# JingyunLiang/HCFlow

Measured on AMD Instinct MI355X. Metric: HR images/sec (inverse sample) DIV2K x4 160px LR, higher is better.
Workload: dtype f32 via f16x3 split (hi/lo f16 products, f32 accumulate); 1 GPU; SR_DF2K_4X inverse sampling (netG reverse=True), batch 16/GPU, LR 160x160 -> HR 640x640, tau=0.8, eps on device, output all-gather over RCCL for N>1; global_batch=16, lr_size=160, parallelism=dp1, streams_per_gpu=2

## Files before the change

### hcflow_amd/_lib.py

```python
from __future__ import annotations

import ctypes as C
import os
from typing import List, Optional, Sequence, Tuple

import torch

_HERE = os.path.dirname(os.path.abspath(__file__))
LIB_PATH = os.environ.get("HCFLOW_LIB", os.path.join(_HERE, "libhcflow_hip.so"))

HCF_OK = 0
ERR_NAMES = {-1: "HCF_ERR_ARG", -2: "HCF_ERR_HIP", -3: "HCF_ERR_STATE", -4: "HCF_ERR_KEY",
             -5: "HCF_ERR_SHAPE", -6: "HCF_ERR_UNSUPPORTED", -7: "HCF_ERR_NOMEM"}
FLAG_NO_CLAMP = 1
FLAG_NO_RANGE_CHECK = 2
FLAG_KEEP_COND = 4
FLAG_REUSE_COND = 8
DATA_LAUNCH_BATCH = 64

SYMBOLS = [
    "hcf_create", "hcf_destroy", "hcf_last_error", "hcf_param_count", "hcf_param_info",
    "hcf_set_param", "hcf_finalize", "hcf_inverse", "hcf_inverse_ex", "hcf_check_range", "hcf_check_range_samples", "hcf_aux_stream", "hcf_forward_sr", "hcf_forward_rescale",
    "hcf_encode_sr",
    "hcf_workspace_bytes", "hcf_weight_bytes", "hcf_profile_convs", "hcf_conv_time_ms",
# ... 5 lines not shown
    "hcf_train_forward_sr", "hcf_train_backward", "hcf_train_backward_phase", "hcf_bind_param_device", "hcf_refresh_from_device",
    "hcf_train_inverse", "hcf_train_backward_inverse", "hcf_metric_psnr_ssim", "hcf_metric_imresize_down",
    "hcf_train_select_tape", "hcf_train_forward_rescale", "hcf_train_backward_rescale",
    "hcf_debug_range_probe", "hcf_debug_range_probe_read", "hcf_debug_conv_plan",
    "hcf_aux_conv2d_workspace", "hcf_aux_conv2d", "hcf_aux_conv2d_backward", "hcf_adam_step",
    "hcf_lpips_workspace", "hcf_lpips_alex", "hcf_lpips_backward_workspace", "hcf_lpips_alex_backward",
    "hcf_aux_bn_act_workspace", "hcf_aux_bn_act", "hcf_aux_bn_act_backward",
    "hcf_op_step_forward_backward", "hcf_op_step_inverse_backward", "hcf_op_prior_backward", "hcf_op_quant_logp_backward",
    "hcf_op_output_grad_backward", "hcf_op_conv_epilogue_backward", "hcf_op_lu_chain",
    "hcf_train_backward_inverse_ex", "hcf_train_backward_counts", "hcf_op_prior_sample_backward",
    "hcf_aux_input_norm", "hcf_aux_input_norm_backward", "hcf_aux_maxpool2", "hcf_aux_maxpool2_act_backward",
    "hcf_aux_act_backward", "hcf_aux_feature_loss_workspace", "hcf_aux_feature_loss",
    "hcf_train_backward_ex", "hcf_train_backward_rescale_ex", "hcf_train_encode_sr", "hcf_train_backward_encode",
    "hcf_op_quant_logp_backward_lr", "hcf_op_prior_encode_logp_backward", "hcf_op_input_grad",
    "hcf_data_prepare_batch", "hcf_data_prepare_paired",
    "hcf_op_fcn12", "hcf_op_conv2d_step_inverse",
]


class HcfError(RuntimeError):
    pass


class hcf_config(C.Structure):
    _fields_ = [
        ("kind", C.c_int32), ("scale", C.c_int32), ("in_nc", C.c_int32), ("quant", C.c_float),
        ("L", C.c_int32), ("K", C.c_int32 * 4), ("after", C.c_int32 * 4), ("squeeze", C.c_int32),
        ("perm", C.c_int32), ("coupling", C.c_int32), ("nn_module", C.c_int32), ("hidden", C.c_int32),
        ("c_perm", C.c_int32), ("c_coupling", C.c_int32), ("c_nn_module", C.c_int32), ("c_hidden", C.c_int32),
        ("rrdb_nb", C.c_int32 * 2), ("rrdb_nf", C.c_int32), ("rrdb_gc", C.c_int32),
        ("lu_decomposed", C.c_int32),
# ... 90 lines not shown
    lib.hcf_refresh_from_device.argtypes = [vp, vp]
    lib.hcf_train_forward_sr.argtypes = [vp, fp, fp, fp, fp, fp, fp, i32, i32, i32, vp]
    lib.hcf_train_backward.argtypes = [vp, f32, fp, i64, vp]
    lib.hcf_train_backward_phase.argtypes = [vp, i32, f32, fp, i64, vp]
    lib.hcf_train_backward_ex.argtypes = [vp, f32, fp, i64, fp, fp, vp]
    lib.hcf_train_backward_rescale_ex.argtypes = [vp, fp, fp, fp, fp, i64, fp, vp]
    lib.hcf_train_encode_sr.argtypes = [vp, fp, fp, fp, C.POINTER(fp), i32, fp, i32, i32, i32, u32, vp]
    lib.hcf_train_backward_encode.argtypes = [vp, fp, C.POINTER(fp), i32, fp, fp, i64, fp, vp]
    lib.hcf_op_quant_logp_backward_lr.argtypes = [fp, fp, fp, fp, i32, i32, i32, f32, vp]
    lib.hcf_op_prior_encode_logp_backward.argtypes = [fp, fp, fp, fp, fp, fp, i32, i32, i32, i32, i32, f32, vp]
    lib.hcf_op_input_grad.argtypes = [fp, fp, i32, i32, i32, i32, i32, vp]
    lib.hcf_actnorm_init_request.argtypes = [vp, C.POINTER(C.c_char_p), i32]
    lib.hcf_get_param.argtypes = [vp, C.c_char_p, fp, i64]
    lib.hcf_op_conv2d.argtypes = [C.POINTER(fp), C.POINTER(i32), C.POINTER(i32), i32, i32, i32, i32, fp, fp, fp,
                                  i32, i32, i32, fp, f32, fp, f32, fp, vp]
    lib.hcf_op_conv2d_backward.argtypes = [C.POINTER(fp), C.POINTER(i32), C.POINTER(i32), i32, i32, i32, i32, fp, i32, i32,
                                           fp, C.POINTER(fp), fp, fp, vp]
    lib.hcf_op_fcn12.argtypes = [C.POINTER(fp), C.POINTER(i32), C.POINTER(i32), i32, i32, i32, i32, fp, fp, fp, fp, fp, fp, fp, fp, i32,
                                 C.POINTER(i32), vp]
    lib.hcf_op_conv2d_step_inverse.argtypes = [fp, i32, fp, fp, fp, i32, fp, i32, i32, i32, fp, fp, fp, fp, fp, i32, i32, i32, i32,
                                               C.POINTER(i32), vp]
    lib.hcf_op_squeeze2d.argtypes = [fp, fp, i32, i32, i32, i32, i32, vp]
    lib.hcf_op_unsqueeze2d.argtypes = [fp, fp, i32, i32, i32, i32, i32, vp]
    lib.hcf_op_step_inverse.argtypes = [fp, fp, fp, i32, i32, i32, i32, i32, i32, i32, fp, fp, fp, vp]
    lib.hcf_op_step_forward_head.argtypes = [fp, fp, i32, i32, i32, i32, fp, fp, fp, vp]
    lib.hcf_op_step_forward_couple.argtypes = [fp, fp, fp, fp, i32, i32, i32, i32, i32, i32, i32, vp]
    lib.hcf_op_gauss_logp.argtypes = [fp, fp, fp, i32, i32, i32, i32, vp]
    lib.hcf_op_gauss_sample.argtypes = [fp, fp, f32, u64, fp, i32, i32, i32, i32, i32, vp]
    lib.hcf_op_step_forward_backward.argtypes = [fp] * 8 + [i32] * 7 + [fp, fp, f32, vp]
    lib.hcf_op_step_inverse_backward.argtypes = [fp] * 10 + [i32] * 7 + [fp, fp, fp, vp]
# ... 186 lines not shown
```

### hcflow_amd/csrc/hcf_common.h

```cpp
#pragma once
#include <hip/hip_runtime.h>
#include <vector>
#include <stdint.h>

#define HCF_OK 0
#define HCF_ERR_ARG (-1)
#define HCF_ERR_HIP (-2)
#define HCF_ERR_STATE (-3)
#define HCF_ERR_KEY (-4)
#define HCF_ERR_SHAPE (-5)
#define HCF_ERR_UNSUPPORTED (-6)
#define HCF_ERR_NOMEM (-7)

namespace hcf {

struct View {
  float* p;
  int cs;
  int c0;
  int n;
  int up;
};

static inline View mkview(float* p, int cs, int c0, int n, int up = 0) {
// ... 34 lines not shown
int conv_f16x3_scaled_blocks(int B, int H, int W, int* strip_w = nullptr, int* tile_h = nullptr);

enum { ACT_NONE = 0, ACT_RELU = 1, ACT_LRELU = 2 };
__device__ __forceinline__ float act_slope(int act) { return act == ACT_RELU ? 0.f : act == ACT_LRELU ? 0.2f : 1.f; }
__device__ __forceinline__ float apply_act(float v, float slope) {
  const float lo = (slope == 0.f) ? -3.0e38f : -INFINITY;
  return !(v <= 0.f) ? v : slope * fmaxf(v, lo);
}
enum { PREC_EXACT = 0, PREC_F16X3 = 1 };

int launch_conv(const ConvArgs& a, int taps, hipStream_t st);
int launch_conv_f16x3(const ConvArgs& a, int taps, hipStream_t st);
int launch_fcn12(const ConvArgs& a, hipStream_t st, unsigned* grid_out = nullptr, int* ntiles_out = nullptr);
size_t pack_conv_weights_wino(const float* w, int cin, int cout, const int* srcs, int nsrc, std::vector<float>& out, int min_cin = -1);
size_t pack_conv_weights_1x1_frag(const float* w, std::vector<float>& out);
int launch_conv_wino(const ConvArgs& a, const void* wpack_wino, hipStream_t st);
int wino_clock_probe(int enable);
double wino_clock_probe_mhz();
int conv_wino_grid(int B, int H, int W, int ntile_n);
bool conv_wino_rounds_ok(int B, int H, int W, int ntile_n);
int launch_repack_wino(const float* w_dev, int cin, int cout, int cout_tile, void* pk, hipStream_t st);
struct RepackWinoJob { const float* w; void* pk; int cin, cout, cout_tile; long long blk0;
                       const float* w2; int split, ld, ld2, z1_n, z1_pad, frag1x1;
                       int tr, k0, kn, tr_off; };
int launch_repack_wino_batch(const RepackWinoJob* jobs_dev, int njobs, long long nblocks, hipStream_t st);

struct WgradArgs {
  View src[kMaxSrc];
  int nsrc;
  View g;
  int B, H, W;
// ... 189 lines not shown
```

### hcflow_amd/csrc/hcf_conv_wino.h

```cpp
#pragma once
#include <hip/hip_runtime.h>
#include <stdint.h>
#include <string.h>
#include <math.h>
#include <type_traits>
#include <vector>

namespace hcf {
namespace wino {

constexpr int TW = 32, TH = 8, HWP = TW + 2, HHP = TH + 2;
constexpr int A_REAL_PIECES = HHP * HWP * 4;
constexpr int A_BYTES = 22 * 1024;
constexpr int W_BYTES = 16 * 2 * 2 * 32 * 16;
constexpr int STAGE = A_BYTES + W_BYTES;
constexpr int X_BYTES = 10240;
constexpr int S0_OFF = 0, X_OFF = STAGE, S1_OFF = STAGE + X_BYTES, TAB_OFF = S1_OFF + STAGE;
constexpr int LDS_BYTES = TAB_OFF + 512;
constexpr float UNSPLIT = 1.f / 2048.f;

struct Src { const float* p; int cs, c0, n; };
struct Args {
  Src src[3];
  int nsrc;
// ... 7 lines not shown
  const float* res1; int res1_cs, res1_c0; float rs1;
  const float* res2; int res2_cs, res2_c0; float rs2;
  float* out2; int out2_cs, out2_c0, act2;
  int out2_split;
  const float* pre; int pre_cs, pre_c0;
  const char* f_w;
  const float* f_bias; const float* f_scale; int f_act;
  const float* in_max;
  const float* fb_y; int fb_y_cs, fb_y_c0;
  int fb_act;
  float* fb_part; float* fb_max; float* fb_max2;
  int* ovf;
  const char* zeros;
  int rev;
  int top_wait;
  unsigned long long* dbg;
  unsigned long long* clk;
};

static inline bool pack_weights_wino(const float* w, int cin, int cout, std::vector<uint16_t>& pk) {
#pragma clang fp contract(off)
  static const double G[4][3] = {{1, 0, 0}, {.5, .5, .5}, {.5, -.5, .5}, {0, 0, 1}};
  const int nchunk = cin / 16, ntn = (cout + 31) / 32;
  pk.assign(((size_t)ntn * nchunk + 1) * (W_BYTES / 2), 0);
  for (int oc = 0; oc < cout; ++oc)
    for (int ic = 0; ic < cin; ++ic) {
      const float* g = w + ((size_t)oc * cin + ic) * 9;
      double t[4][3], U[4][4];
      for (int i = 0; i < 4; ++i)
        for (int j = 0; j < 3; ++j) t[i][j] = G[i][0] * g[0 * 3 + j] + G[i][1] * g[1 * 3 + j] + G[i][2] * g[2 * 3 + j];
// ... 149 lines not shown
}

typedef uint32_t u32x2 __attribute__((ext_vector_type(2)));
__device__ __forceinline__ void split4(const f32x4& v, u32x2& h, u32x2& l) {
#pragma unroll
  for (int i = 0; i < 2; ++i) {
    const f16x2 hh = {(_Float16)v[2 * i], (_Float16)v[2 * i + 1]};
    h[i] = __builtin_bit_cast(uint32_t, hh);
    uint32_t lo;
    asm("v_fma_mixlo_f16 %0, %1, -1.0, %2 op_sel_hi:[1,0,0]" : "=v"(lo) : "v"(h[i]), "v"(v[2 * i]));
    asm("v_fma_mixhi_f16 %0, %1, -1.0, %2 op_sel:[1,0,0] op_sel_hi:[1,0,0]" : "+v"(lo) : "v"(h[i]), "v"(v[2 * i + 1]));
    l[i] = lo;
  }
}

template <int RES, bool SC = false>
__global__ __launch_bounds__(512, 1) void conv_wino2_kernel(const Args a, const int nunits) {
  using namespace v2;
  extern __shared__ __attribute__((aligned(16))) char lds[];
  const int tid = threadIdx.x, lane = tid & 63, half = lane >> 5, li = lane & 31;
  const int wave = __builtin_amdgcn_readfirstlane(tid >> 6);
  const int xp = wave & 1, tg = wave >> 1;
  const int H = a.H, W = a.W, ntn = a.ntile_n, nchunk = a.nchunk;
  const int tiles_x = (W + TW - 1) / TW, tiles_y = (H + TH2 - 1) / TH2;

  const bool w7 = (wave == 7);
  const int padpix = a.B * H * W;
  int upix[5];
#pragma unroll
  for (int j = 0; j < 5; ++j) upix[j] = padpix;
  uint32_t partpk = 0;
#pragma unroll
  for (int j = 0; j < 5; ++j) {
    const int pa_ = (8 * j + wave) * 64 + lane, hy_ = (pa_ * 241) >> 15, q_ = pa_ - hy_ * 136, m_ = q_ >> 4;
    partpk |= (uint32_t)(((q_ & 15) ^ (m_ & 7)) & 3) << (4 + 2 * j);
  }
  const int k0 = __builtin_amdgcn_readfirstlane(a.src[0].n >> 4);
  const int k1 = k0 + __builtin_amdgcn_readfirstlane(a.nsrc > 1 ? (a.src[1].n >> 4) : 0);
// ... 37 lines not shown
  {                                                                                                \
    const int sidx_ = (uc < k0) ? 0 : (uc < k1) ? 1 : 2;                                           \
    csb_ = sidx_ == 0 ? csb0 : sidx_ == 1 ? csb1 : csb2;                                           \
    rsa_ = sidx_ == 0 ? rs0 : sidx_ == 1 ? rs1 : rs2;                                              \
    so_ = (sidx_ == 0 ? cb0 + uc * 64 : sidx_ == 1 ? cb1 + (uc - k0) * 64 : cb2 + (uc - k1) * 64); \
    ws_ = (unt * nchunk + uc) * W_BYTES;                                                           \
    pp_ = partpk;                                                                                  \
    asm volatile("" : "+v"(pp_));            \
  }
#define W2_A_SLOT(J, DST)                                                                          \
  {                                                                                                \
    const int p16_ = (int)((pp_ >> (2 * (J))) & 0x30u);                                            \
    const int vo_ = (int)__umul24((unsigned)upix[J], (unsigned)csb_) + p16_;                       \
    W2_DMA(rsa_, vo_, so_, DST);                                                                   \
  }
#define W2_ISSUE(J0, J1, STG)                                                                      \
  {                                                                                                \
    char* const sb_ = lds + (STG) * STAGE2 + wave * 1024;                                          \
    _Pragma("unroll") for (int j_ = (J0); j_ < (J1); ++j_) {                                       \
      if (j_ < 4) W2_A_SLOT(j_ < 5 ? j_ : 0, sb_ + j_ * 8192)                                      \
      else if (j_ == 4) { if (!w7) W2_A_SLOT(4, sb_ + 4 * 8192) else W2_DMA(rsw, wvo, ws_, sb_ + 4 * 8192); } \
      else if (j_ < 8) W2_DMA(rsw, wvo, ws_ + (8 * j_ + wave - 39) * 1024, sb_ + j_ * 8192);       \
      else if (!w7) W2_DMA(rsw, wvo, ws_ + (8 * 8 + wave - 39) * 1024, sb_ + 8 * 8192);            \
    }                                                                                              \
  }

  const int trow = li >> 4, tcol = li & 15;
  int poff[4];
#pragma unroll
  for (int j = 0; j < 4; ++j) poff[j] = a2_off(4 * tg + 2 * trow, 2 * tcol + j, 2 * half);
  const int rowP = xp ? ROWB : 0, rowS = xp ? 3 * ROWB : 2 * ROWB;
  const float sg = __builtin_bit_cast(float, __builtin_amdgcn_readfirstlane(__builtin_bit_cast(int, xp ? -1.f : 1.f)));
  const int fw = A2_BYTES + half * 512 + li * 16 + xp * (8 * 4 * 512);

  float in_s = 1.f, out_s = 1.f;
  int in_max_bits = 0;
// ... 7 lines not shown
  }
  if (FBK) {
    if (fb) {
      *reinterpret_cast<f32x4*>(lds + FB2_OFF + tid * 16) = f32x4{0.f, 0.f, 0.f, 0.f};
      if (tid == 0) *reinterpret_cast<int*>(lds + FB2_OFF + 512 * 16) = 0;
    }
  }
  int u = blockIdx.x;
  if (u >= nunits) return;
#if defined(WINO_PROF)
  unsigned long long pw[8] = {0, 0, 0, 0, 0, 0, 0, 0};
  const unsigned long long pw_t0 = __builtin_readcyclecounter();
#endif
  W2_SETUP_UNIT(u)
  W2_CHUNK_SCALARS()
  W2_ISSUE(0, 9, 0)
  ++uc;
  int g = 0;
  const float slope = a.act == 1 ? 0.f : a.act == 2 ? 0.2f : 1.f;

  while (true) {
    f32x16 acc[8];
#pragma unroll
    for (int p = 0; p < 8; ++p)
#pragma unroll
      for (int r = 0; r < 16; ++r) acc[p][r] = 0.f;
    const int eb = ub, ey0 = uy0, ex0 = ux0, ent = unt;
    const int un = u + gridDim.x;

    for (int c = 0; c < nchunk; ++c, ++g) {
      const int stg = g & 1;
#if defined(WINO_PROF)
      const unsigned long long q0 = __builtin_readcyclecounter();
#endif
      asm volatile("s_waitcnt vmcnt(0)" ::: "memory");
#if defined(WINO_PROF)
      const unsigned long long q1 = __builtin_readcyclecounter();
#endif
      __builtin_amdgcn_s_barrier();
#if defined(WINO_PROF)
      const unsigned long long q2 = __builtin_readcyclecounter();
      pw[0] += q1 - q0; pw[1] += q2 - q1;
#endif
      if (c + 1 == nchunk) {
        if (un < nunits) W2_SETUP_UNIT(un)
        else {
          uc = 0; unt = 0;
#pragma unroll
          for (int j = 0; j < 5; ++j) upix[j] = padpix;
        }
      }
      W2_CHUNK_SCALARS()
      const char* const sb = lds + stg * STAGE2;
      const int so = stg ^ 1;
#define W2_LOAD_ROW(D, OFF)                                                                        \
  _Pragma("unroll") for (int j = 0; j < 4; ++j) {                                                  \
    const f32x4 x0_ = *reinterpret_cast<const f32x4*>(sb + poff[j] + (OFF));                       \
    const f32x4 x1_ = *reinterpret_cast<const f32x4*>(sb + (poff[j] ^ 16) + (OFF));                \
    _Pragma("unroll") for (int k = 0; k < 4; ++k) { D[j][k] = x0_[k]; D[j][4 + k] = x1_[k]; }      \
  }
#define W2_V(NU, T, K) (((NU) == 0) ? T[0][K] - T[2][K] : ((NU) == 1) ? T[1][K] + T[2][K] : ((NU) == 2) ? T[1][K] - T[2][K] : T[1][K] - T[3][K])
#define W2_MFMA(P, WW, VX) acc[P] = __builtin_amdgcn_mfma_f32_32x32x16_f16(WW, __builtin_bit_cast(f16x8, VX), acc[P], 0, 0, 0);
#define W2_XI(I, T)                                                                                \
  _Pragma("unroll") for (int nu = 0; nu < 4; ++nu) {                                               \
    float v_[8];                                                                                   \
    _Pragma("unroll") for (int k = 0; k < 8; ++k) v_[k] = W2_V(nu, T, k);                          \
    u32x4 vh_, vl_;                                                                                \
    if (SC) split8s(v_, in_s, vh_, vl_); else split8(v_, vh_, vl_);                                \
    const f16x8 w1_ = *reinterpret_cast<const f16x8*>(sb + fw + (((I) * 4 + nu) * 4) * 512);       \
    const f16x8 w2_ = *reinterpret_cast<const f16x8*>(sb + fw + (((I) * 4 + nu) * 4 + 2) * 512);   \
    W2_MFMA((I) * 4 + nu, w1_, vh_)                                                                \
    W2_MFMA((I) * 4 + nu, w2_, vh_)                                                                \
    W2_MFMA((I) * 4 + nu, w1_, vl_)                                                                \
  }
      float t_[4][8];
      {
        float ra[4][8], rc[4][8];
        W2_LOAD_ROW(ra, rowP)
        W2_LOAD_ROW(rc, 2 * ROWB)
        W2_ISSUE(0, 3, so)
#pragma unroll
        for (int j = 0; j < 4; ++j)
#pragma unroll
          for (int k = 0; k < 8; ++k) t_[j][k] = ra[j][k] - rc[j][k];
      }
      W2_XI(0, t_)
      W2_ISSUE(3, 6, so)
      {
        float ra[4][8], rc[4][8];
        W2_LOAD_ROW(ra, ROWB)
        W2_LOAD_ROW(rc, rowS)
#pragma unroll
        for (int j = 0; j < 4; ++j)
#pragma unroll
          for (int k = 0; k < 8; ++k) t_[j][k] = fmaf(sg, rc[j][k], ra[j][k]);
      }
      W2_ISSUE(6, 9, so)
      ++uc;
      W2_XI(1, t_)
#if defined(WINO_PROF)
      pw[6] += __builtin_readcyclecounter() - q2;
#endif
#undef W2_XI
#undef W2_MFMA
#undef W2_V
#undef W2_LOAD_ROW
    }

#if defined(WINO_PROF)
    const unsigned long long qe0 = __builtin_readcyclecounter();
#endif
    float chk = 0.f;
    f32x4 fbs = {0.f, 0.f, 0.f, 0.f};
    float fbm = 0.f;
    const float fb_neg = a.fb_act == 1 ? 0.f : a.fb_act == 2 ? 0.2f : 1.f;
    {
      char* const xbuf = lds + ((g - 1) & 1) * STAGE2 + tg * 16384;
      const int p8 = lane >> 3, qd = (lane >> 1) & 3, hd = lane & 1;
      const int wpos = (half * 32 + ((li + 4 * half) & 31)) * 16;
      const int wpos1 = (half * 32 + ((li + 4 * half + 8) & 31)) * 16;
      const int cb = ent * 32 + 8 * qd + 4 * hd;
      const f32x4 bs = *reinterpret_cast<const f32x4*>(lds + TAB2_OFF + cb * 4);
      const f32x4 ms = *reinterpret_cast<const f32x4*>(lds + TAB2_OFF + 256 + cb * 4);
      const bool second = (RES == 0) && a.out2 != nullptr && cb >= a.out2_split;
      const float slope_l = second ? (a.act2 == 1 ? 0.f : a.act2 == 2 ? 0.2f : 1.f) : slope;
      __builtin_amdgcn_s_barrier();
#pragma unroll
      for (int oa = 0; oa < 2; ++oa) {
        f32x4 rv1[2][2], rv2[2][2];
        size_t pixs[2][2];
        bool oks[2][2];
        int rpos[2];
// ... 636 lines not shown
  if (a.res1 && (((a.res1_cs | a.res1_c0) & 3) || (reinterpret_cast<uintptr_t>(a.res1) & 15))) return -6;
  if (a.res2 && (((a.res2_cs | a.res2_c0) & 3) || (reinterpret_cast<uintptr_t>(a.res2) & 15))) return -6;
  if (a.res2 && !a.res1) return -1;
  if ((long long)a.B * a.H * a.W >= (1LL << 24)) return -6;
  if (version == 4 && (a.ntile_n != 2 || a.cout > 64)) return -6;
  if (version == 4) {
    const int cs_[4] = {a.out_cs, a.out2 ? a.out2_cs : 0, a.res1 ? a.res1_cs : 0, a.res2 ? a.res2_cs : 0};
    for (int i = 0; i < 4; ++i)
      if (cs_[i] < 0 || (long long)(a.W + 1) * cs_[i] >= 0x7fffffffLL) return -6;
  }
  const int th = (version == 2) ? v2::TH2 : (version == 4) ? v4::TH4 : TH;
  const int tiles_x = (a.W + TW - 1) / TW, tiles_y = (a.H + th - 1) / th;
  const long long nunits = (long long)a.B * tiles_x * tiles_y * (version == 4 ? 1 : a.ntile_n);
  if (nunits < 1 || nunits > 0x7fffffffLL) return -1;
  const unsigned grid = (unsigned)(nunits < ncu ? nunits : ncu);
  static bool attr_dev[64][3][8] = {};
  int dev_ = 0;
  if (hipGetDevice(&dev_) != hipSuccess || dev_ < 0 || dev_ >= 64) return -2;
  bool (&attr)[3][8] = attr_dev[dev_];
  if (a.pre && (version != 2 || a.res1 || a.res2 || ((a.pre_cs | a.pre_c0) & 3) || (reinterpret_cast<uintptr_t>(a.pre) & 15))) return -6;
  if (a.out2 && (a.res1 || a.pre || ((a.out2_cs | a.out2_c0) & 3) || (reinterpret_cast<uintptr_t>(a.out2) & 15))) return -6;
  if (a.out2 && version != 4 && (version != 2 || a.ntile_n != 1 || a.out2_split != 16)) return -6;
  if (a.f_w && (version != 4 || a.res1 || a.res2 || a.out2 || !a.f_bias || !a.f_scale || (reinterpret_cast<uintptr_t>(a.f_w) & 15))) return -6;
  const int res = (a.pre || a.f_w) ? 3 : a.res2 ? 2 : a.res1 ? 1 : 0;
  const bool sc = a.in_max != nullptr;
  if (sc && (res > 1 || a.out2 || (version != 2 && version != 4))) return -6;
  if (a.fb_y && (!sc || version != 2 || res != 0 || a.ntile_n != 1 || !a.fb_part || ((a.fb_y_cs | a.fb_y_c0) & 3) ||
                 (reinterpret_cast<uintptr_t>(a.fb_y) & 15))) return -6;
  const int ldsb = (version == 2) ? (sc ? v2::LDS2S_BYTES : v2::LDS2_BYTES) : (version == 4) ? v4::LDS4_BYTES : LDS_BYTES;
  const int vi = (version == 2) ? 1 : (version == 4) ? 2 : 0;
  const int ai = res + (sc ? 4 : 0);
  auto go = [&](auto fn, int threads) {
    if (!attr[vi][ai]) {
      if (hipFuncSetAttribute(reinterpret_cast<const void*>(fn), hipFuncAttributeMaxDynamicSharedMemorySize, ldsb) != hipSuccess) return -2;
      attr[vi][ai] = true;
    }
    hipLaunchKernelGGL(fn, dim3(grid), dim3(threads), ldsb, st, a, (int)nunits);
    return hipGetLastError() == hipSuccess ? 0 : -2;
  };
  if (sc && version == 4) return res == 0 ? go(conv_wino4_kernel<0, true>, 512) : go(conv_wino4_kernel<1, true>, 512);
  if (sc && version == 2) return res == 0 ? go(conv_wino2_kernel<0, true>, 512) : go(conv_wino2_kernel<1, true>, 512);
  if (version == 4) {
    if (res == 0) return go(conv_wino4_kernel<0>, 512);
    if (res == 1) return go(conv_wino4_kernel<1>, 512);
    if (res == 3) return go(conv_wino4_kernel<3>, 512);
    return go(conv_wino4_kernel<2>, 512);
  }
  if (version == 2) {
    if (res == 0) return go(conv_wino2_kernel<0>, 512);
    if (res == 1) return go(conv_wino2_kernel<1>, 512);
    if (res == 3) return go(conv_wino2_kernel<3>, 512);
    return go(conv_wino2_kernel<2>, 512);
  }
  return -6;
}
#endif

}
}
```

### hcflow_amd/csrc/hcf_conv_wino.hip

```cpp
#include "hcf_common.h"
#include <cstdlib>
#include "hcf_conv_wino.h"
#include "hcf_pack_index.h"
#include <atomic>

namespace hcf {

size_t pack_conv_weights_wino(const float* w, int cin, int cout, const int* srcs, int nsrc, std::vector<float>& out, int min_cin_arg) {
  out.clear();
  static const int min_cin_env = getenv("HCF_WINO_MIN_CIN") ? atoi(getenv("HCF_WINO_MIN_CIN")) : 64;
  const int min_cin = min_cin_arg >= 0 ? min_cin_arg : min_cin_env;
  if (!w || cin < min_cin || (cout != 32 && cout != 64) || nsrc < 1 || nsrc > 3) return 0;
  int sum = 0;
  for (int i = 0; i < nsrc; ++i) {
    if (srcs[i] < 16 || (srcs[i] & 15)) return 0;
    sum += srcs[i];
  }
  if (sum != cin) return 0;
  std::vector<uint16_t> pk;
  if (!(cout == 64 ? wino::pack_weights_wino64(w, cin, cout, pk) : wino::pack_weights_wino(w, cin, cout, pk))) return 0;
  out.resize((pk.size() * 2 + 3) / 4);
  memcpy(out.data(), pk.data(), pk.size() * 2);
  return pk.size() * 2;
}
// ... 111 lines not shown
long long wino_units(int B, int H, int W, int ntile_n) {
  return (long long)B * ((W + 31) / 32) * ((ntile_n == 2) ? (H + 7) / 8 : (H + 15) / 16);
}
int conv_wino_grid(int B, int H, int W, int ntile_n) {
  const long long nunits = wino_units(B, H, W, ntile_n);
  const int ncu = wino_ncu();
  return (int)(nunits < ncu ? nunits : ncu);
}
bool conv_wino_rounds_ok(int B, int H, int W, int ntile_n) {
  const int ncu = wino_ncu();
  const long long nunits = wino_units(B, H, W, ntile_n);
  const long long rounds = (nunits + ncu - 1) / ncu;
  return !(rounds >= 2 && nunits * 100 < rounds * ncu * 75) && (long long)B * H * W < (1LL << 24);
}

int launch_conv_wino(const ConvArgs& a, const void* wpack_wino, hipStream_t st) {
  if (!wpack_wino || a.nsrc < 1 || a.nsrc > 3 || a.w2 || a.tC > 0) return HCF_ERR_UNSUPPORTED;
  wino::Args w;
  memset(&w, 0, sizeof(w));
  int cin = 0;
  for (int i = 0; i < a.nsrc; ++i) {
    if (a.src[i].up != 0) return HCF_ERR_UNSUPPORTED;
    w.src[i] = wino::Src{a.src[i].p, a.src[i].cs, a.src[i].c0, a.src[i].n};
    cin += a.src[i].n;
  }
  for (int i = a.nsrc; i < 3; ++i) w.src[i] = w.src[0];
  w.nsrc = a.nsrc;
  w.B = a.B; w.H = a.H; w.W = a.W;
  w.wpack = reinterpret_cast<const char*>(wpack_wino);
  w.nchunk = cin / 16;
  w.ntile_n = a.wino_ntile > 0 ? a.wino_ntile : a.out.n / 32;
// ... 17 lines not shown
  }
  w.in_max = a.in_max;
  if (a.fb_y.p) {
    if (!a.in_max || a.fb_scale || a.fb_zy || a.fb_max2 == a.in_max || !a.fb_part || a.res1.p || a.res2.p || w.ntile_n != 1) return HCF_ERR_UNSUPPORTED;
    w.fb_y = a.fb_y.p; w.fb_y_cs = a.fb_y.cs; w.fb_y_c0 = a.fb_y.c0; w.fb_act = a.fb_act;
    w.fb_part = a.fb_part; w.fb_max = a.fb_max; w.fb_max2 = a.fb_max2;
  }
  w.ovf = a.ovf;
  w.zeros = reinterpret_cast<const char*>(a.zeros);
  if (g_wino_clk_on) {
    int dev_ = 0;
    if (hipGetDevice(&dev_) == hipSuccess && dev_ >= 0 && dev_ < 64) w.clk = g_wino_clk[dev_];
  }
  static const int top_wait = getenv("HCF_WINO_TOP_WAIT") ? atoi(getenv("HCF_WINO_TOP_WAIT")) : 0;
  w.top_wait = top_wait;
  const char* const rev_env = getenv("HCF_WINO_REV");
  const int rev_mode = rev_env ? atoi(rev_env) : 1;
  static thread_local unsigned rev_flip = 0;
  w.rev = rev_mode ? (int)(rev_flip++ & 1u) : 0;
  const int ncu = wino_ncu();
  if (!conv_wino_rounds_ok(a.B, a.H, a.W, w.ntile_n)) return HCF_ERR_UNSUPPORTED;
  const int r = wino::launch(w, ncu, st, w.ntile_n == 2 ? 4 : 2);
  return r == 0 ? HCF_OK : r == -6 ? HCF_ERR_UNSUPPORTED : r == -2 ? HCF_ERR_HIP : HCF_ERR_ARG;
}

}
```

### hcflow_amd/csrc/hcf_engine_run.inc

```

  hipStream_t st = nullptr;
  bool dry() const { return arena.dry; }

  struct Buf {
    float* p; int C; int cs;
    View v(int c0, int n, int up = 0) const { return mkview(p, cs, c0, n, up); }
    View all() const { return mkview(p, cs, 0, C, 0); }
  };
  Buf alloc(int B, int H, int W, int C) {
    Buf b;
    b.C = C;
    b.cs = ru4(C);
    b.p = arena.alloc((size_t)B * H * W * b.cs);
    return b;
  }

  int B_ = 0;

  bool can_fuse_fcn(const Conv& c1, const Conv& c2, const View* z1 = nullptr) const {
    static const bool off = getenv("HCF_NO_FUSE_FCN") != nullptr;
    if (off) return false;
    if (taping) return false;
    if (z1 && ((z1->cs | z1->c0) & 3) != 0) return false;
    return use_f16 && c1.wpack16 && c2.wpack16 && c1.taps == 9 && c2.taps == 1 && c1.cout == 64 && c2.cout == 64 &&
// ... 315 lines not shown
    if (partial && s.mode == CPL_AFFINE) {
      a.partial = partial + pslot;
      a.partial_stride = pstride;
      pslot += step_blocks_per_sample(H, W);
    }
    HCF_LAUNCH(launch_step_couple_fwd(a, st));
  }

  bool tape_fat = false;
  void run_rdb(const Rdb& r, View xin, const Buf& grow, int H, int W, View out, View res2, float rs2, const Buf* fatp = nullptr) {
    const int gc = cfg.rrdb_gc;
    const bool fat_ok = fatp && fatp->p && use_f16 && (!taping || tape_fat) && !(g_f16x3_ablation & 256) &&
                        (gc == 16 || conv_wino_rounds_ok(B_, H, W, 2)) && conv_wino_rounds_ok(B_, H, W, 1) &&
                        wino_offsets_ok(H, W, std::max(std::max(xin.cs, grow.cs), fatp->cs));
    static const long long fat12_pixels = getenv("HCF_FAT12_PIXELS") ? atoll(getenv("HCF_FAT12_PIXELS")) : 40000;
    const bool use_fat[2] = {fat_ok && r.fat[0] && (gc == 16 || (long long)H * W <= fat12_pixels), fat_ok && r.fat[1]};
    ConvOpt last;
    last.res1 = xin; last.rs1 = 0.2f; last.res2 = res2; last.rs2 = rs2;
    if (use_fat[0] || use_fat[1]) {
      for (int j = 0; j < 2; ++j) {
        std::vector<View> srcs;
        srcs.push_back(xin);
        if (j > 0) srcs.push_back(grow.v(0, 2 * j * gc));
        if (use_fat[j]) {
          const FatExtra fa = {fatp->v(0, gc), ACT_NONE, false};
          ConvOpt oa; oa.fat = &fa;
          run_conv(r.ca[j], srcs, H, W, grow.v(2 * j * gc, gc), oa);
          const FatExtra fb = {View(), ACT_NONE, true};
          ConvOpt ob; ob.res1 = fatp->v(0, gc); ob.fat = &fb;
          run_conv(r.cb[j], {grow.v(2 * j * gc, gc)}, H, W, grow.v((2 * j + 1) * gc, gc), ob);
        } else {
// ... 305 lines not shown
```

### hcflow_amd/csrc/hcf_ops.hip

```cpp
#include <math.h>
#include <string.h>

#include <vector>

#include "../../include/hcflow.h"
#include "hcf_common.h"

namespace hcf {
void pack_conv_weights(const float* w, int cin, int cout, int taps, const int* srcs, int nsrc, std::vector<float>& pk,
                       int& nchunk, int& npad);
bool pack_conv_weights_f16x3(const float* w, int cin, int cout, int taps, const int* srcs, int nsrc,
                             std::vector<float>& pk_as_float, int& nchunk, int& npad);
static int g_op_precision = PREC_EXACT;
static double g_last_clock_mhz = 0;
extern int g_f16x3_ablation;

static inline int ru4(int c) { return (c + 3) & ~3; }

struct Tmp {
  std::vector<void*> ptrs;
  bool ok = true;
  float* dev(size_t nfloat) {
    void* p = nullptr;
    if (hipMalloc(&p, nfloat * sizeof(float) + 256) != hipSuccess) { ok = false; return nullptr; }
// ... 129 lines not shown
  a.res2 = mkview(nullptr, 0, 0, 0);
  if (res1) { a.res1 = nhwc_from_nchw(t, res1, B, cout, H, W, st, rc); a.rs1 = rs1; }
  if (res2) { a.res2 = nhwc_from_nchw(t, res2, B, cout, H, W, st, rc); a.rs2 = rs2; }
  if (!t.ok) return HCF_ERR_NOMEM;
  if (rc != HCF_OK) return rc;
  rc = pack_and_launch(t, a, w, cin, cout, k, srcs, n_src, st);
  if (rc != HCF_OK) return rc;
  rc = launch_nhwc_to_nchw(a.out, out, B, cout, H, W, 0, st);
  if (hipStreamSynchronize(st) != hipSuccess) return HCF_ERR_HIP;
  if (a.ovf) {
    int h = 0;
    if (hipMemcpy(&h, a.ovf, sizeof(int), hipMemcpyDeviceToHost) != hipSuccess) return HCF_ERR_HIP;
    if (h) return HCF_ERR_UNSUPPORTED;
  }
  return rc;
}

static void transpose_weights(const float* w, int cin, int cout, int taps, int off, int n, std::vector<float>& wt) {
  wt.assign((size_t)n * cout * taps, 0.f);
  for (int ic = 0; ic < n; ++ic)
    for (int oc = 0; oc < cout; ++oc)
      for (int t = 0; t < taps; ++t)
        wt[((size_t)ic * cout + oc) * taps + t] = w[((size_t)oc * cin + off + ic) * taps + (taps - 1 - t)];
}

int hcf_op_conv2d_backward(const float* const* src, const int32_t* src_c, const int32_t* src_up, int32_t n_src,
                           int32_t B, int32_t H, int32_t W, const float* w, int32_t cout, int32_t k, const float* g,
                           float* const* dsrc, float* dw, float* dbias, hcf_stream_t stream) {
  if (!src || !src_c || !w || !g || n_src < 1 || n_src > kMaxSrc || (k != 1 && k != 3) || cout < 1 || cout > 96)
    return HCF_ERR_ARG;
// ... 853 lines not shown
```

### hcflow_amd/ops.py

```python
from __future__ import annotations

import ctypes as C
from typing import Optional, Sequence

import torch

from . import _lib


def _dev(t: torch.Tensor) -> torch.Tensor:
    if t.device.type != "cuda":
        raise _lib.HcfError("hcflow_amd ops need CUDA (MI355X) tensors")
    return t.detach().to(torch.float32).contiguous()


def _host(t: Optional[torch.Tensor]) -> Optional[torch.Tensor]:
    return None if t is None else t.detach().to("cpu", torch.float32).contiguous()


ACT = {None: 0, "none": 0, "relu": 1, "lrelu": 2}


def set_precision(mode: str):
    _lib.check(_lib.load().hcf_op_set_precision(_lib.Engine.PRECISIONS[mode]), None, "hcf_op_set_precision")
# ... 4 lines not shown
    srcs = [_dev(s) for s in srcs]
    n = len(srcs)
    ups = list(ups) if ups is not None else [0] * n
    B = srcs[0].shape[0]
    H, W = srcs[0].shape[2] << ups[0], srcs[0].shape[3] << ups[0]
    cout, cin, k, _ = weight.shape
    assert sum(s.shape[1] for s in srcs) == cin
    ptrs = (C.c_void_p * n)(*[s.data_ptr() for s in srcs])
    cs = (C.c_int32 * n)(*[s.shape[1] for s in srcs])
    us = (C.c_int32 * n)(*ups)
    out = torch.empty(B, cout, H, W, device=srcs[0].device)
    r1 = _dev(res1) if res1 is not None else None
    r2 = _dev(res2) if res2 is not None else None
    _lib.launch("hcf_op_conv2d", out.device, ptrs, cs, us, n, B, H, W, _host(weight), _host(bias), _host(scale), cout, k, ACT[act],
                r1, float(rs1), r2, float(rs2), out)
    return out


def conv2d_backward(srcs: Sequence[torch.Tensor], weight: torch.Tensor, grad_out: torch.Tensor,
                    ups: Optional[Sequence[int]] = None, need_input_grads: bool = True):
    srcs = [_dev(s) for s in srcs]
    g = _dev(grad_out)
    n = len(srcs)
    ups = list(ups) if ups is not None else [0] * n
    B, cout, H, W = g.shape
    co, cin, k, _ = weight.shape
    assert co == cout and sum(s.shape[1] for s in srcs) == cin
    ptrs = (C.c_void_p * n)(*[s.data_ptr() for s in srcs])
    cs = (C.c_int32 * n)(*[s.shape[1] for s in srcs])
    us = (C.c_int32 * n)(*ups)
# ... 237 lines not shown
```

### include/hcflow.h

```cpp
#ifndef HCFLOW_H_
#define HCFLOW_H_

#include <stddef.h>
#include <stdint.h>

#ifdef __cplusplus
extern "C" {
#endif

#define HCF_OK 0
#define HCF_ERR_ARG (-1)
#define HCF_ERR_HIP (-2)
#define HCF_ERR_STATE (-3)
#define HCF_ERR_KEY (-4)
#define HCF_ERR_SHAPE (-5)
#define HCF_ERR_UNSUPPORTED (-6)
#define HCF_ERR_NOMEM (-7)

#define HCF_KIND_SR 0
#define HCF_KIND_RESCALING 1
#define HCF_SQUEEZE_CHECKERBOARD 0
#define HCF_SQUEEZE_HAAR 1
#define HCF_PERM_INVCONV 0
#define HCF_PERM_NONE 1
// ... 108 lines not shown
  uint32_t offset;
  uint32_t n;
} hcf_adam_chunk;
int hcf_adam_step(float* param, float* exp_avg, float* exp_avg_sq, const hcf_adam_chunk* chunks_dev, int32_t n_chunks,
                  double lr, double beta1, double beta2, double eps, double weight_decay, int64_t step, hcf_stream_t stream);

int hcf_metric_psnr_ssim(const float* gt, const float* sr, int32_t B, int32_t H, int32_t W, int32_t crop_border,
                         int32_t scale, double* out, hcf_stream_t stream);
int hcf_metric_imresize_down(const float* x, int32_t B, int32_t H, int32_t W, int32_t scale, double* out,
                             hcf_stream_t stream);

int hcf_op_conv2d(const float* const* src, const int32_t* src_c, const int32_t* src_up, int32_t n_src, int32_t B,
                  int32_t H, int32_t W, const float* w, const float* bias, const float* scale, int32_t cout, int32_t k,
                  int32_t act, const float* res1, float rs1, const float* res2, float rs2, float* out,
                  hcf_stream_t stream);

int hcf_op_conv2d_backward(const float* const* src, const int32_t* src_c, const int32_t* src_up, int32_t n_src,
                           int32_t B, int32_t H, int32_t W, const float* w, int32_t cout, int32_t k, const float* g,
                           float* const* dsrc, float* dw, float* dbias, hcf_stream_t stream);

int hcf_op_squeeze2d(const float* x, float* out, int32_t B, int32_t C, int32_t H, int32_t W, int32_t haar, hcf_stream_t stream);
int hcf_op_unsqueeze2d(const float* x, float* out, int32_t B, int32_t C4, int32_t H, int32_t W, int32_t haar, hcf_stream_t stream);
int hcf_op_step_inverse(const float* z, const float* h, float* out, int32_t B, int32_t C, int32_t H, int32_t W,
                        int32_t hC, int32_t mode, int32_t ns, const float* mat, const float* an_bias,
                        const float* an_logs, hcf_stream_t stream);
int hcf_op_step_forward_head(const float* z, float* out, int32_t B, int32_t C, int32_t H, int32_t W, const float* mat,
                             const float* an_bias, const float* an_logs, hcf_stream_t stream);
int hcf_op_step_forward_couple(const float* z, const float* h, float* out, float* logdet, int32_t B, int32_t C,
                               int32_t H, int32_t W, int32_t hC, int32_t mode, int32_t ns, hcf_stream_t stream);
int hcf_op_fcn12(const float* const* src, const int32_t* src_c, const int32_t* src_up, int32_t n_src, int32_t B, int32_t H,
// ... 111 lines not shown
```

Baseline: 134.9 HR images/s.

## Keep Winograd conv weights resident in LDS for two-chunk single-tile-n case

Adds a resident-weight variant of the v2 Winograd conv kernel, used when nchunk==2 and ntile_n==1. Each chunk gets a fixed LDS stage and the weight DMA is skipped on the last chunk, so weights need not be reloaded per unit. The kernel is on by default through an env knob. Also adds a standalone wino32 conv op for testing and ablation flags that can disable this path and the fat12 path. The trade-off is a fixed stage assignment that may reduce overlap, and correctness depends on the weights staying valid in LDS across units.

```diff
diff --git a/hcflow_amd/_lib.py b/hcflow_amd/_lib.py
--- a/hcflow_amd/_lib.py
+++ b/hcflow_amd/_lib.py
@@ -43,7 +43,7 @@
     "hcf_train_backward_ex", "hcf_train_backward_rescale_ex", "hcf_train_encode_sr", "hcf_train_backward_encode",
     "hcf_op_quant_logp_backward_lr", "hcf_op_prior_encode_logp_backward", "hcf_op_input_grad",
     "hcf_data_prepare_batch", "hcf_data_prepare_paired",
-    "hcf_op_fcn12", "hcf_op_conv2d_step_inverse",
+    "hcf_op_fcn12", "hcf_op_conv2d_step_inverse", "hcf_op_conv2d_wino32",
 ]
 
 
@@ -164,6 +164,7 @@
     lib.hcf_get_param.argtypes = [vp, C.c_char_p, fp, i64]
     lib.hcf_op_conv2d.argtypes = [C.POINTER(fp), C.POINTER(i32), C.POINTER(i32), i32, i32, i32, i32, fp, fp, fp,
                                   i32, i32, i32, fp, f32, fp, f32, fp, vp]
+    lib.hcf_op_conv2d_wino32.argtypes = [C.POINTER(fp), C.POINTER(i32), i32, i32, i32, i32, fp, fp, fp, i32, fp, fp, vp]
     lib.hcf_op_conv2d_backward.argtypes = [C.POINTER(fp), C.POINTER(i32), C.POINTER(i32), i32, i32, i32, i32, fp, i32, i32,
                                            fp, C.POINTER(fp), fp, fp, vp]
     lib.hcf_op_fcn12.argtypes = [C.POINTER(fp), C.POINTER(i32), C.POINTER(i32), i32, i32, i32, i32, fp, fp, fp, fp, fp, fp, fp, fp, i32,
diff --git a/hcflow_amd/csrc/hcf_common.h b/hcflow_amd/csrc/hcf_common.h
--- a/hcflow_amd/csrc/hcf_common.h
+++ b/hcflow_amd/csrc/hcf_common.h
@@ -72,7 +72,7 @@
 int launch_fcn12(const ConvArgs& a, hipStream_t st, unsigned* grid_out = nullptr, int* ntiles_out = nullptr);
 size_t pack_conv_weights_wino(const float* w, int cin, int cout, const int* srcs, int nsrc, std::vector<float>& out, int min_cin = -1);
 size_t pack_conv_weights_1x1_frag(const float* w, std::vector<float>& out);
-int launch_conv_wino(const ConvArgs& a, const void* wpack_wino, hipStream_t st);
+int launch_conv_wino(const ConvArgs& a, const void* wpack_wino, hipStream_t st, bool any_rounds = false);
 int wino_clock_probe(int enable);
 double wino_clock_probe_mhz();
 int conv_wino_grid(int B, int H, int W, int ntile_n);
diff --git a/hcflow_amd/csrc/hcf_conv_wino.h b/hcflow_amd/csrc/hcf_conv_wino.h
--- a/hcflow_amd/csrc/hcf_conv_wino.h
+++ b/hcflow_amd/csrc/hcf_conv_wino.h
@@ -45,6 +45,7 @@
   const char* zeros;
   int rev;
   int top_wait;
+  int resident_w;
   unsigned long long* dbg;
   unsigned long long* clk;
 };
@@ -224,14 +225,14 @@
   }
 }
 
-template <int RES, bool SC = false>
+template <int RES, bool SC = false, bool RW = false>
 __global__ __launch_bounds__(512, 1) void conv_wino2_kernel(const Args a, const int nunits) {
   using namespace v2;
   extern __shared__ __attribute__((aligned(16))) char lds[];
   const int tid = threadIdx.x, lane = tid & 63, half = lane >> 5, li = lane & 31;
   const int wave = __builtin_amdgcn_readfirstlane(tid >> 6);
   const int xp = wave & 1, tg = wave >> 1;
-  const int H = a.H, W = a.W, ntn = a.ntile_n, nchunk = a.nchunk;
+  const int H = a.H, W = a.W, ntn = RW ? 1 : a.ntile_n, nchunk = RW ? 2 : a.nchunk;
   const int tiles_x = (W + TW - 1) / TW, tiles_y = (H + TH2 - 1) / TH2;
 
   const bool w7 = (wave == 7);
@@ -299,12 +300,13 @@
     const int vo_ = (int)__umul24((unsigned)upix[J], (unsigned)csb_) + p16_;                       \
     W2_DMA(rsa_, vo_, so_, DST);                                                                   \
   }
-#define W2_ISSUE(J0, J1, STG)                                                                      \
+#define W2_ISSUE(J0, J1, STG, NOW)                                                                    \
   {                                                                                                \
     char* const sb_ = lds + (STG) * STAGE2 + wave * 1024;                                          \
     _Pragma("unroll") for (int j_ = (J0); j_ < (J1); ++j_) {                                       \
       if (j_ < 4) W2_A_SLOT(j_ < 5 ? j_ : 0, sb_ + j_ * 8192)                                      \
-      else if (j_ == 4) { if (!w7) W2_A_SLOT(4, sb_ + 4 * 8192) else W2_DMA(rsw, wvo, ws_, sb_ + 4 * 8192); } \
+      else if (j_ == 4) { if (!w7) W2_A_SLOT(4, sb_ + 4 * 8192) else if (!(NOW)) W2_DMA(rsw, wvo, ws_, sb_ + 4 * 8192); } \
+      else if (NOW) { }                                                                            \
       else if (j_ < 8) W2_DMA(rsw, wvo, ws_ + (8 * j_ + wave - 39) * 1024, sb_ + j_ * 8192);       \
       else if (!w7) W2_DMA(rsw, wvo, ws_ + (8 * 8 + wave - 39) * 1024, sb_ + 8 * 8192);            \
     }                                                                                              \
@@ -342,11 +344,12 @@
 #endif
   W2_SETUP_UNIT(u)
   W2_CHUNK_SCALARS()
-  W2_ISSUE(0, 9, 0)
+  W2_ISSUE(0, 9, 0, false)
   ++uc;
   int g = 0;
   const float slope = a.act == 1 ? 0.f : a.act == 2 ? 0.2f : 1.f;
 
+  constexpr int CHUNK_UNROLL = RW ? 2 : 1;
   while (true) {
     f32x16 acc[8];
 #pragma unroll
@@ -356,8 +359,9 @@
     const int eb = ub, ey0 = uy0, ex0 = ux0, ent = unt;
     const int un = u + gridDim.x;
 
+#pragma unroll CHUNK_UNROLL
     for (int c = 0; c < nchunk; ++c, ++g) {
-      const int stg = g & 1;
+      const int stg = RW ? c : (g & 1);
 #if defined(WINO_PROF)
       const unsigned long long q0 = __builtin_readcyclecounter();
 #endif
@@ -381,6 +385,7 @@
       W2_CHUNK_SCALARS()
       const char* const sb = lds + stg * STAGE2;
       const int so = stg ^ 1;
+      const bool now = RW && (c + 1 == nchunk);
 #define W2_LOAD_ROW(D, OFF)                                                                        \
   _Pragma("unroll") for (int j = 0; j < 4; ++j) {                                                  \
     const f32x4 x0_ = *reinterpret_cast<const f32x4*>(sb + poff[j] + (OFF));                       \
@@ -406,14 +411,14 @@
         float ra[4][8], rc[4][8];
         W2_LOAD_ROW(ra, rowP)
         W2_LOAD_ROW(rc, 2 * ROWB)
-        W2_ISSUE(0, 3, so)
+        W2_ISSUE(0, 3, so, now)
 #pragma unroll
         for (int j = 0; j < 4; ++j)
 #pragma unroll
           for (int k = 0; k < 8; ++k) t_[j][k] = ra[j][k] - rc[j][k];
       }
       W2_XI(0, t_)
-      W2_ISSUE(3, 6, so)
+      W2_ISSUE(3, 6, so, now)
       {
         float ra[4][8], rc[4][8];
         W2_LOAD_ROW(ra, ROWB)
@@ -423,7 +428,7 @@
 #pragma unroll
           for (int k = 0; k < 8; ++k) t_[j][k] = fmaf(sg, rc[j][k], ra[j][k]);
       }
-      W2_ISSUE(6, 9, so)
+      W2_ISSUE(6, 9, so, now)
       ++uc;
       W2_XI(1, t_)
 #if defined(WINO_PROF)
@@ -443,7 +448,7 @@
     float fbm = 0.f;
     const float fb_neg = a.fb_act == 1 ? 0.f : a.fb_act == 2 ? 0.2f : 1.f;
     {
-      char* const xbuf = lds + ((g - 1) & 1) * STAGE2 + tg * 16384;
+      char* const xbuf = lds + (RW ? 1 : ((g - 1) & 1)) * STAGE2 + tg * 16384;
       const int p8 = lane >> 3, qd = (lane >> 1) & 3, hd = lane & 1;
       const int wpos = (half * 32 + ((li + 4 * half) & 31)) * 16;
       const int wpos1 = (half * 32 + ((li + 4 * half + 8) & 31)) * 16;
@@ -1110,10 +1115,10 @@
   const long long nunits = (long long)a.B * tiles_x * tiles_y * (version == 4 ? 1 : a.ntile_n);
   if (nunits < 1 || nunits > 0x7fffffffLL) return -1;
   const unsigned grid = (unsigned)(nunits < ncu ? nunits : ncu);
-  static bool attr_dev[64][3][8] = {};
+  static bool attr_dev[64][3][12] = {};
   int dev_ = 0;
   if (hipGetDevice(&dev_) != hipSuccess || dev_ < 0 || dev_ >= 64) return -2;
-  bool (&attr)[3][8] = attr_dev[dev_];
+  bool (&attr)[3][12] = attr_dev[dev_];
   if (a.pre && (version != 2 || a.res1 || a.res2 || ((a.pre_cs | a.pre_c0) & 3) || (reinterpret_cast<uintptr_t>(a.pre) & 15))) return -6;
   if (a.out2 && (a.res1 || a.pre || ((a.out2_cs | a.out2_c0) & 3) || (reinterpret_cast<uintptr_t>(a.out2) & 15))) return -6;
   if (a.out2 && version != 4 && (version != 2 || a.ntile_n != 1 || a.out2_split != 16)) return -6;
@@ -1125,7 +1130,8 @@
                  (reinterpret_cast<uintptr_t>(a.fb_y) & 15))) return -6;
   const int ldsb = (version == 2) ? (sc ? v2::LDS2S_BYTES : v2::LDS2_BYTES) : (version == 4) ? v4::LDS4_BYTES : LDS_BYTES;
   const int vi = (version == 2) ? 1 : (version == 4) ? 2 : 0;
-  const int ai = res + (sc ? 4 : 0);
+  const bool rw = version == 2 && !sc && a.resident_w && a.nchunk == 2 && a.ntile_n == 1;
+  const int ai = res + (sc ? 4 : rw ? 8 : 0);
   auto go = [&](auto fn, int threads) {
     if (!attr[vi][ai]) {
       if (hipFuncSetAttribute(reinterpret_cast<const void*>(fn), hipFuncAttributeMaxDynamicSharedMemorySize, ldsb) != hipSuccess) return -2;
@@ -1142,6 +1148,12 @@
     if (res == 3) return go(conv_wino4_kernel<3>, 512);
     return go(conv_wino4_kernel<2>, 512);
   }
+  if (rw) {
+    if (res == 0) return go(conv_wino2_kernel<0, false, true>, 512);
+    if (res == 1) return go(conv_wino2_kernel<1, false, true>, 512);
+    if (res == 3) return go(conv_wino2_kernel<3, false, true>, 512);
+    return go(conv_wino2_kernel<2, false, true>, 512);
+  }
   if (version == 2) {
     if (res == 0) return go(conv_wino2_kernel<0>, 512);
     if (res == 1) return go(conv_wino2_kernel<1>, 512);
diff --git a/hcflow_amd/csrc/hcf_conv_wino.hip b/hcflow_amd/csrc/hcf_conv_wino.hip
--- a/hcflow_amd/csrc/hcf_conv_wino.hip
+++ b/hcflow_amd/csrc/hcf_conv_wino.hip
@@ -5,6 +5,8 @@
 #include <atomic>
 
 namespace hcf {
+
+extern int g_f16x3_ablation;
 
 size_t pack_conv_weights_wino(const float* w, int cin, int cout, const int* srcs, int nsrc, std::vector<float>& out, int min_cin_arg) {
   out.clear();
@@ -149,7 +151,7 @@
   return !(rounds >= 2 && nunits * 100 < rounds * ncu * 75) && (long long)B * H * W < (1LL << 24);
 }
 
-int launch_conv_wino(const ConvArgs& a, const void* wpack_wino, hipStream_t st) {
+int launch_conv_wino(const ConvArgs& a, const void* wpack_wino, hipStream_t st, bool any_rounds) {
   if (!wpack_wino || a.nsrc < 1 || a.nsrc > 3 || a.w2 || a.tC > 0) return HCF_ERR_UNSUPPORTED;
   wino::Args w;
   memset(&w, 0, sizeof(w));
@@ -197,12 +199,14 @@
   }
   static const int top_wait = getenv("HCF_WINO_TOP_WAIT") ? atoi(getenv("HCF_WINO_TOP_WAIT")) : 0;
   w.top_wait = top_wait;
+  static const int resident_w = getenv("HCF_WINO_RESIDENT_W") ? atoi(getenv("HCF_WINO_RESIDENT_W")) : 1;
+  w.resident_w = resident_w && !(g_f16x3_ablation & 4096);
   const char* const rev_env = getenv("HCF_WINO_REV");
   const int rev_mode = rev_env ? atoi(rev_env) : 1;
   static thread_local unsigned rev_flip = 0;
-  w.rev = rev_mode ? (int)(rev_flip++ & 1u) : 0;
+  w.rev = rev_mode == 2 ? 1 : rev_mode ? (int)(rev_flip++ & 1u) : 0;
   const int ncu = wino_ncu();
-  if (!conv_wino_rounds_ok(a.B, a.H, a.W, w.ntile_n)) return HCF_ERR_UNSUPPORTED;
+  if (!any_rounds && !conv_wino_rounds_ok(a.B, a.H, a.W, w.ntile_n)) return HCF_ERR_UNSUPPORTED;
   const int r = wino::launch(w, ncu, st, w.ntile_n == 2 ? 4 : 2);
   return r == 0 ? HCF_OK : r == -6 ? HCF_ERR_UNSUPPORTED : r == -2 ? HCF_ERR_HIP : HCF_ERR_ARG;
 }
diff --git a/hcflow_amd/csrc/hcf_engine_run.inc b/hcflow_amd/csrc/hcf_engine_run.inc
--- a/hcflow_amd/csrc/hcf_engine_run.inc
+++ b/hcflow_amd/csrc/hcf_engine_run.inc
@@ -353,7 +353,8 @@
                         (gc == 16 || conv_wino_rounds_ok(B_, H, W, 2)) && conv_wino_rounds_ok(B_, H, W, 1) &&
                         wino_offsets_ok(H, W, std::max(std::max(xin.cs, grow.cs), fatp->cs));
     static const long long fat12_pixels = getenv("HCF_FAT12_PIXELS") ? atoll(getenv("HCF_FAT12_PIXELS")) : 40000;
-    const bool use_fat[2] = {fat_ok && r.fat[0] && (gc == 16 || (long long)H * W <= fat12_pixels), fat_ok && r.fat[1]};
+    const bool use_fat[2] = {fat_ok && r.fat[0] && (gc == 16 || ((long long)H * W <= fat12_pixels && !(g_f16x3_ablation & 8192))),
+                             fat_ok && r.fat[1]};
     ConvOpt last;
     last.res1 = xin; last.rs1 = 0.2f; last.res2 = res2; last.rs2 = rs2;
     if (use_fat[0] || use_fat[1]) {
diff --git a/hcflow_amd/csrc/hcf_ops.hip b/hcflow_amd/csrc/hcf_ops.hip
--- a/hcflow_amd/csrc/hcf_ops.hip
+++ b/hcflow_amd/csrc/hcf_ops.hip
@@ -167,6 +167,55 @@
     if (h) return HCF_ERR_UNSUPPORTED;
   }
   return rc;
+}
+
+int hcf_op_conv2d_wino32(const float* const* src, const int32_t* src_c, int32_t n_src, int32_t B, int32_t H, int32_t W,
+                         const float* w, const float* bias, const float* scale, int32_t act, const float* pre, float* out,
+                         hcf_stream_t stream) {
+  if (!src || !src_c || !w || !out || n_src < 1 || n_src > kMaxSrc || B < 1 || H < 1 || W < 1) return HCF_ERR_ARG;
+  hipStream_t st = (hipStream_t)stream;
+  const int cout = 32;
+  Tmp t;
+  int rc = HCF_OK;
+  ConvArgs a;
+  memset(&a, 0, sizeof(a));
+  int cin = 0;
+  int srcs[kMaxSrc];
+  for (int i = 0; i < n_src; ++i) {
+    a.src[i] = nhwc_from_nchw(t, src[i], B, src_c[i], H, W, st, rc);
+    srcs[i] = src_c[i];
+    cin += src_c[i];
+  }
+  for (int i = n_src; i < kMaxSrc; ++i) a.src[i] = a.src[0];
+  a.nsrc = n_src;
+  a.B = B; a.H = H; a.W = W;
+  std::vector<float> hb(cout, 0.f), hs(cout, 1.f);
+  for (int n = 0; n < cout; ++n) {
+    if (bias) hb[n] = bias[n];
+    if (scale) hs[n] = scale[n];
+  }
+  a.bias = t.up(hb);
+  a.scale = t.up(hs);
+  a.act = act;
+  a.out = mkview(t.dev((size_t)B * H * W * cout), cout, 0, cout);
+  a.res1 = mkview(nullptr, 0, 0, 0);
+  a.res2 = mkview(nullptr, 0, 0, 0);
+  if (pre) { a.res1 = nhwc_from_nchw(t, pre, B, cout, H, W, st, rc); a.res1_pre = 1; }
+  a.ovf = (int*)t.dev(64);
+  if (a.ovf && hipMemsetAsync(a.ovf, 0, 256, st) != hipSuccess) return HCF_ERR_HIP;
+  a.zeros = reinterpret_cast<const float*>(a.ovf) + 16;
+  std::vector<float> pkw;
+  if (!pack_conv_weights_wino(w, cin, cout, srcs, n_src, pkw, 16)) return HCF_ERR_UNSUPPORTED;
+  const float* wino = t.up(pkw);
+  if (!t.ok) return HCF_ERR_NOMEM;
+  if (rc != HCF_OK) return rc;
+  rc = launch_conv_wino(a, wino, st, true);
+  if (rc != HCF_OK) return rc;
+  rc = launch_nhwc_to_nchw(a.out, out, B, cout, H, W, 0, st);
+  if (hipStreamSynchronize(st) != hipSuccess) return HCF_ERR_HIP;
+  int h = 0;
+  if (hipMemcpy(&h, a.ovf, sizeof(int), hipMemcpyDeviceToHost) != hipSuccess) return HCF_ERR_HIP;
+  return h ? HCF_ERR_UNSUPPORTED : rc;
 }
 
 static void transpose_weights(const float* w, int cin, int cout, int taps, int off, int n, std::vector<float>& wt) {
diff --git a/hcflow_amd/ops.py b/hcflow_amd/ops.py
--- a/hcflow_amd/ops.py
+++ b/hcflow_amd/ops.py
@@ -42,6 +42,20 @@
     r2 = _dev(res2) if res2 is not None else None
     _lib.launch("hcf_op_conv2d", out.device, ptrs, cs, us, n, B, H, W, _host(weight), _host(bias), _host(scale), cout, k, ACT[act],
                 r1, float(rs1), r2, float(rs2), out)
+    return out
+
+
+def conv2d_wino32(srcs: Sequence[torch.Tensor], weight: torch.Tensor, bias=None, scale=None, act=None, pre=None) -> torch.Tensor:
+    srcs = [_dev(s) for s in srcs]
+    n = len(srcs)
+    B, _, H, W = srcs[0].shape
+    cout, cin, k, _ = weight.shape
+    assert cout == 32 and k == 3 and sum(s.shape[1] for s in srcs) == cin
+    ptrs = (C.c_void_p * n)(*[s.data_ptr() for s in srcs])
+    cs = (C.c_int32 * n)(*[s.shape[1] for s in srcs])
+    out = torch.empty(B, cout, H, W, device=srcs[0].device)
+    _lib.launch("hcf_op_conv2d_wino32", out.device, ptrs, cs, n, B, H, W, _host(weight), _host(bias), _host(scale), ACT[act],
+                _dev(pre) if pre is not None else None, out)
     return out
 
 
diff --git a/include/hcflow.h b/include/hcflow.h
--- a/include/hcflow.h
+++ b/include/hcflow.h
@@ -146,6 +146,9 @@
                   int32_t H, int32_t W, const float* w, const float* bias, const float* scale, int32_t cout, int32_t k,
                   int32_t act, const float* res1, float rs1, const float* res2, float rs2, float* out,
                   hcf_stream_t stream);
+int hcf_op_conv2d_wino32(const float* const* src, const int32_t* src_c, int32_t n_src, int32_t B, int32_t H, int32_t W,
+                         const float* w, const float* bias, const float* scale, int32_t act, const float* pre, float* out,
+                         hcf_stream_t stream);
 
 int hcf_op_conv2d_backward(const float* const* src, const int32_t* src_c, const int32_t* src_up, int32_t n_src,
                            int32_t B, int32_t H, int32_t W, const float* w, int32_t cout, int32_t k, const float* g,
```

Result: no change. 135.0 HR images/s (median of 2 runs) (+0.1%).
